# atx/padne

Hardware: AMD Instinct MI355X
Metric: CG solves/s (higher is better)
Workload: dtype f64; 1 GPU; C4 8-layer N=10M: 8-layer jittered triangular Laplacian, 9999392 nodes, via-ring stitched, 1 A source/sink, amg-PCG to rtol 1e-12; n_unknowns=9999391, nnz_per_rank=69955225, rows_per_rank=9999391, parallelism=layer-partitioned x1

## Files before the change

padne_amd/csrc/amg.hip:

```cpp
#include "common.hpp"

#include <functional>
#include <type_traits>
#include <memory>

#include <algorithm>
#include <chrono>
#include <math.h>
#include <stdlib.h>
#include <string.h>

namespace padne {

struct AmgLevel {
    const padne_csr *A = nullptr;
    padne_csr *A_owned = nullptr;
    padne_csr *P = nullptr;
    padne_csr *R = nullptr;
    padne_csr *W = nullptr;
    double lambda = 2.0;
    double jac = 0.0;
    long long n = 0;
    double *b = nullptr, *xa = nullptr, *xb = nullptr, *tmp = nullptr;
    float *b8 = nullptr, *xa8 = nullptr, *xb8 = nullptr, *tmp8 = nullptr;
// ... 183 lines not shown
            const double sgm = (off + fabs(dF)) / fabs(dF);
            my_max = sgm > my_max ? sgm : my_max;
            const double plain = abs_all * fabs(di);
            my_plain = plain > my_plain ? plain : my_plain;
        }
    }
    if (bound_partial != nullptr) {
        for (int o = 32; o > 0; o >>= 1) {
            my_max = fmax(my_max, __shfl_down(my_max, o, 64));
            my_plain = fmax(my_plain, __shfl_down(my_plain, o, 64));
        }
        if (lane == 0) {
            red[w] = my_max;
            red2[w] = my_plain;
        }
        __syncthreads();
        if (threadIdx.x == 0) {
            bound_partial[blockIdx.x] = fmax(fmax(red[0], red[1]), fmax(red[2], red[3]));
            bound_partial[kMaxPartials + blockIdx.x] = fmax(fmax(red2[0], red2[1]), fmax(red2[2], red2[3]));
        }
    }
}

template <typename T>
__global__ __launch_bounds__(256) void nbr_max(int n, int n_wtiles, const int *__restrict__ srow,
                                               const int *__restrict__ scol, const T *__restrict__ in,
                                               T *__restrict__ out) {
    constexpr int CH = 512;
    __shared__ T park_all[4 * CH];
    const int lane = threadIdx.x & 63, w = threadIdx.x >> 6;
    T *park = park_all + w * CH;
    const XcdSweep sw = xcd_sweep(n_wtiles, 4, w);
    for (long long wt = sw.t0; wt < sw.t1; wt += sw.stride) {
        const int row0 = (int)wt * 64;
        const int row1 = min(row0 + 64, n);
        const int r = row0 + lane;
        int rs = 0, re = 0;
        T m = 0;
        if (r < row1) {
            rs = srow[r];
            re = srow[r + 1];
            m = in[r];
        }
        const int k0 = __shfl(rs, 0, 64);
        const int k1 = __shfl(re, row1 - row0 - 1, 64);
        for (int base = k0; base < k1; base += CH) {
#pragma unroll
            for (int j = 0; j < CH / 64; ++j) {
                const int e = base + lane + 64 * j;
                park[lane + 64 * j] = (e < k1) ? in[scol[e]] : (T)0;
            }
            asm volatile("s_waitcnt lgkmcnt(0)" ::: "memory");
            __builtin_amdgcn_wave_barrier();
            const int lo = max(rs, base), hi = min(re, base + CH);
            for (int k = lo; k < hi; ++k) {
                const T v = park[k - base];
                m = v > m ? v : m;
            }
            asm volatile("" ::: "memory");
            __builtin_amdgcn_wave_barrier();
        }
        if (r < row1) out[r] = m;
    }
}

template <typename T>
__global__ __launch_bounds__(256) void nbr_max_wpr(int n, const int *__restrict__ srow, const int *__restrict__ scol,
                                                   const T *__restrict__ in, T *__restrict__ out) {
    const int lane = threadIdx.x & 63;
    const long long r = (long long)blockIdx.x * 4 + (threadIdx.x >> 6);
    if (r >= n) return;
    const int rs = srow[r], re = srow[r + 1];
    T m = in[r];
    for (int k = rs + lane; k < re; k += 64) {
        const T v = in[scol[k]];
        m = v > m ? v : m;
    }
#pragma unroll
    for (int off = 32; off > 0; off >>= 1) {
        const T o = __shfl_down(m, off, 64);
        m = o > m ? o : m;
    }
    if (lane == 0) out[r] = m;
}

__device__ __forceinline__ bool mis_decide_one(int i, unsigned int top, unsigned int *__restrict__ word,
                                               signed char *__restrict__ state) {
    const unsigned int mine = word[i];
    if (top == kMisRoot) {
        state[i] = 2;
        word[i] = 0u;
        return false;
    }
    if (top == mine) {
        state[i] = 1;
        word[i] = kMisRoot;
        return false;
    }
    return true;
}

template <typename T, bool DECIDE>
__global__ __launch_bounds__(256) void nbr_max_xw(int n, int n_wtiles, const int *__restrict__ srow,
                                                  const int *__restrict__ scol, const unsigned char *__restrict__ spos,
                                                  const int4 *__restrict__ xw_desc, const int run,
                                                  const T *__restrict__ in, T *__restrict__ out,
                                                  unsigned int *__restrict__ word, signed char *__restrict__ state,
                                                  int *__restrict__ undecided) {
    constexpr int CH = 512;
    __shared__ int open_red[4];
    int open = 0;
    __shared__ T park_all[4 * CH];
    __shared__ T xs_all[4 * 3 * 88];
    const int lane = threadIdx.x & 63, w = threadIdx.x >> 6;
    T *park = park_all + w * CH;
    T *xs = xs_all + w * 3 * 88;
    const XcdSweep sw = xcd_sweep(n_wtiles, 4, w);
    for (long long wt = sw.t0; wt < sw.t1; wt += sw.stride) {
        const int row0 = (int)wt * 64;
        const int row1 = min(row0 + 64, n);
        const int r = row0 + lane;
        int rs = 0, re = 0;
// ... 44 lines not shown
                for (int j = 0; j < CH / 64; ++j) {
                    const int e = base + lane + 64 * j;
                    park[lane + 64 * j] = (e < k1) ? in[scol[e]] : (T)0;
                }
                asm volatile("s_waitcnt lgkmcnt(0)" ::: "memory");
                __builtin_amdgcn_wave_barrier();
                const int lo = max(rs, base), hi = min(re, base + CH);
                for (int k = lo; k < hi; ++k) {
                    const T v = park[k - base];
                    m = v > m ? v : m;
                }
                asm volatile("" ::: "memory");
                __builtin_amdgcn_wave_barrier();
            }
        }
        if (r < row1) {
            if (DECIDE) {
                if (state[r] == 0 && mis_decide_one(r, (unsigned int)m, word, state)) ++open;
            } else {
                out[r] = m;
            }
        }
    }
    if (DECIDE) {
        for (int off = 32; off > 0; off >>= 1) open += __shfl_down(open, off, 64);
        if (lane == 0) open_red[w] = open;
        __syncthreads();
        if (threadIdx.x == 0) {
            const int t = open_red[0] + open_red[1] + open_red[2] + open_red[3];
            if (t) atomicAdd(undecided, t);
        }
    }
}

__global__ void mis_init_words(int n, unsigned int *__restrict__ word, signed char *__restrict__ state,
                               int *__restrict__ counters, int n_counters, unsigned char *__restrict__ pad, int n_pad) {
    const int i = blockIdx.x * blockDim.x + threadIdx.x;
    if (i < n) {
        word[i] = prio32_of(i);
        state[i] = 0;
    }
    if (i < n_counters) counters[i] = 0;
    if (pad != nullptr && i < n_pad) pad[i] = 0;
}

constexpr int kMisTailCap = 512;
__global__ __launch_bounds__(1024) void mis_tail_rounds(const int *__restrict__ cnt_ptr, int *list_a, int *list_b,
// ... 182 lines not shown
            for (int u = 0; u < 8; ++u) aj[u] = (k0 + u < k1 && j[u] != i) ? agg_in[j[u]] : -1;
#pragma unroll
            for (int u = 0; u < 8; ++u) {
                const double w = fabs(v[u]);
                if (aj[u] >= 0 && w > best) {
                    best = w;
                    a = aj[u];
                }
            }
        }
        for (int k = k0 + 8; k < k1; ++k) {
            const int j = scol[k];
            if (j == i) continue;
            const int aj = agg_in[j];
            if (aj < 0) continue;
            const double w = fabs(vals[k]);
            if (w > best) {
                best = w;
                a = aj;
            }
        }
    }
    agg_out[i] = a;
}

__global__ void flag_unaggregated(int n, const int *__restrict__ agg, int *__restrict__ flag) {
    const int i = blockIdx.x * blockDim.x + threadIdx.x;
    if (i < n) flag[i] = agg[i] < 0 ? 1 : 0;
}

__global__ void agg_singletons(int n, const int *__restrict__ scan, const long long *__restrict__ base_dev, int *__restrict__ agg) {
    const int i = blockIdx.x * blockDim.x + threadIdx.x;
    if (i < n && agg[i] < 0) agg[i] = (int)*base_dev + scan[i];
}

__global__ __launch_bounds__(256) void gershgorin_kernel(int n, const int *__restrict__ rowptr,
                                                         const double *__restrict__ vals,
                                                         const double *__restrict__ dinv,
                                                         double *__restrict__ partial_max) {
    __shared__ double red[256];
    double m = 0.0;
    for (int i = blockIdx.x * 256 + threadIdx.x; i < n; i += gridDim.x * 256) {
        double s = 0.0;
        for (int k = rowptr[i]; k < rowptr[i + 1]; ++k) s += fabs(vals[k]);
        s *= fabs(dinv[i]);
        m = s > m ? s : m;
// ... 1459 lines not shown
    PADNE_TRY(sc.alloc(&agg0, (size_t)n));
    PADNE_TRY(sc.alloc(&agg1, (size_t)n));
    constexpr int kMaxRounds = 256;
    PADNE_TRY(sc.alloc(&counter, (size_t)2 * kMaxRounds + 4));
    const dim3 g(nblk(n)), b(256);
    const int *srow = A->rowptr;
    int *scol = nullptr;
    PADNE_TRY(sc.alloc(&scol, (size_t)(A->nnz > 0 ? A->nnz : 1)));
    const int n_wt = (n + 63) / 64;
    int gm_x = std::min(2048, (n_wt + 3) / 4 > 0 ? (n_wt + 3) / 4 : 1);
    if (gm_x >= kNumXcd) gm_x -= gm_x % kNumXcd;
    const dim3 gm((unsigned)gm_x);
    double *bound_part = lambda_f != nullptr ? ctx->partials + 6 * kMaxPartials : nullptr;
    double *bound2 = nullptr;
    if (lambda_f != nullptr) PADNE_TRY(sc.alloc(&bound2, 2));
    const bool xw = A->xw_state == 1 && A->xw_run <= 85;
    unsigned char *spos = nullptr;
    if (xw) {
        PADNE_TRY(sc.alloc(&spos, (size_t)A->nnz + kPadNnz));
    }
    static_assert(kPadNnz >= 2 * kMaxRounds + 4, "one grid for everything the start clears");
    hipLaunchKernelGGL(mis_init_words, dim3(nblk(std::max(n, kPadNnz))), b, 0, s, n, w0, state, counter, 2 * kMaxRounds + 4,
                       spos != nullptr ? spos + A->nnz : (unsigned char *)nullptr, kPadNnz);
    hipLaunchKernelGGL(strength_mark, gm, b, 0, s, n, n_wt, A->rowptr, A->cols, A->vals, A->dinv, theta2, scol, bound_part,
                       xw ? A->xw_desc : (const int4 *)nullptr, xw ? (const unsigned char *)A->xw_lidx : (const unsigned char *)nullptr,
                       xw ? A->xw_run : 0, spos, vals32_out);
    PADNE_HIP_CHECK(hipGetLastError());
    const bool long_rows = !xw && n <= 65536 && A->nnz >= 24LL * n;
    auto launch_round = [&](int *open_counter) {
        if (xw) {
            hipLaunchKernelGGL((nbr_max_xw<unsigned int, false>), gm, b, 0, s, n, n_wt, srow, scol, spos, A->xw_desc, A->xw_run,
                               (const unsigned int *)w0, w1, (unsigned int *)nullptr, (signed char *)nullptr, (int *)nullptr);
            hipLaunchKernelGGL((nbr_max_xw<unsigned int, true>), gm, b, 0, s, n, n_wt, srow, scol, spos, A->xw_desc, A->xw_run,
                               (const unsigned int *)w1, (unsigned int *)nullptr, w0, state, open_counter);
        } else if (long_rows) {
            hipLaunchKernelGGL(nbr_max_wpr<unsigned int>, dim3((unsigned)((n + 3) / 4)), b, 0, s, n, srow, (const int *)scol,
                               (const unsigned int *)w0, w1);
            hipLaunchKernelGGL(nbr_max_wpr<unsigned int>, dim3((unsigned)((n + 3) / 4)), b, 0, s, n, srow, (const int *)scol,
                               (const unsigned int *)w1, w2);
            hipLaunchKernelGGL(mis_decide, dim3(std::min<unsigned>(g.x, 1024u)), b, 0, s, n, w0, w2, state, open_counter);
        } else {
            hipLaunchKernelGGL(nbr_max<unsigned int>, gm, b, 0, s, n, n_wt, srow, scol, w0, w1);
            hipLaunchKernelGGL(nbr_max<unsigned int>, gm, b, 0, s, n, n_wt, srow, scol, w1, w2);
            hipLaunchKernelGGL(mis_decide, dim3(std::min<unsigned>(g.x, 1024u)), b, 0, s, n, w0, w2, state, open_counter);
        }
    };
    if (lambda_f != nullptr)
        hipLaunchKernelGGL(fold_max2_kernel, dim3(1), dim3(256), 0, s, (const double *)bound_part,
                           (const double *)(bound_part + kMaxPartials), (int)gm.x, bound2);
    double h_bound2[2] = {0.0, 0.0};
    bool bound_pending = lambda_f != nullptr;
    auto count_back = [&](const int *dev_count, int *host_count) -> int {
        if (!bound_pending) return read_back(ctx, dev_count, sizeof(int), host_count);
        bound_pending = false;
        return read_back2(ctx, dev_count, sizeof(int), host_count, bound2, sizeof(h_bound2), h_bound2);
    };
    int open_count = n;
    int round = 0;
    const bool compact_ok = A->nnz <= 16LL * n;
    const int full_batch = n > 200000 ? 1 : 4;
    while (round < kMaxRounds && open_count > 0 && (!compact_ok || round < 2 || open_count > n / 8)) {
        const int reps = (round == 0 && compact_ok && full_batch < 2) ? 2 : full_batch;
        for (int rep = 0; rep < reps && round < kMaxRounds; ++rep, ++round) {
            launch_round(counter + round);
        }
        PADNE_HIP_CHECK(hipGetLastError());
        PADNE_TRY(count_back(counter + round - 1, &open_count));
    }
    if (open_count > 0) {
        int *list_a = (int *)w1, *list_b = (int *)w2;
        unsigned int *m2 = nullptr;
        PADNE_TRY(sc.alloc(&m2, (size_t)open_count));
        int *counters = counter + kMaxRounds;
        hipLaunchKernelGGL(mis_collect_open, dim3(std::min<unsigned>(g.x, 1024u)), b, 0, s, n, state, list_a, counters);
        PADNE_HIP_CHECK(hipGetLastError());
        int cnt = open_count, cur = 0;
        while (cur + 1 < kMaxRounds && cnt > 0) {
            if (cnt <= kMisTailCap) {
                hipLaunchKernelGGL(mis_tail_rounds, dim3(1), dim3(1024), 0, s, (const int *)(counters + cur), list_a, list_b, srow,
                                   (const int *)scol, w0, state, m2, counters + cur + 1, kMaxRounds - cur - 1);
                PADNE_HIP_CHECK(hipGetLastError());
                ++cur;
                round += kMaxRounds;
                PADNE_TRY(count_back(counters + cur, &cnt));
                break;
            }
            const dim3 gl(nblk(cnt));
// ... 3 lines not shown
                hipLaunchKernelGGL(mis_decide_list, gl, b, 0, s, counters + cur, list_a, m2, w0, state, list_b, counters + cur + 1);
                std::swap(list_a, list_b);
                ++cur;
            }
            PADNE_HIP_CHECK(hipGetLastError());
            PADNE_TRY(count_back(counters + cur, &cnt));
        }
        open_count = cnt;
    }
    PADNE_REQUIRE(open_count == 0, "independent-set rounds did not terminate");
    if (lambda_f != nullptr) {
        if (bound_pending) PADNE_TRY(read_back(ctx, bound2, sizeof(h_bound2), h_bound2));
        double m = h_bound2[0], mp = h_bound2[1];
        if (!(m > 0.0) || !(m < 1e6)) m = 2.0;
        if (!(mp > 0.0) || !(mp < 1e6)) mp = 2.0;
        *lambda_f = m;
        if (lambda_plain != nullptr) *lambda_plain = mp;
    }
    hipLaunchKernelGGL(flag_state, g, b, 0, s, n, state, flag, 1);
    ScanTicket t_roots, t_single;
    long long h_roots[2] = {0, 0}, h_single[2] = {0, 0};
    PADNE_TRY(scan_i32_begin(ctx, flag, scan, n, &t_roots, true));
    hipLaunchKernelGGL(agg_from_roots, g, b, 0, s, n, state, scan, agg0);
    hipLaunchKernelGGL(agg_join, g, b, 0, s, n, srow, scol, A->vals, agg0, agg1);
    hipLaunchKernelGGL(agg_join, g, b, 0, s, n, srow, scol, A->vals, agg1, agg0);
    hipLaunchKernelGGL(flag_unaggregated, g, b, 0, s, n, agg0, flag);
    int rc_scan = scan_i32_begin(ctx, flag, scan, n, &t_single, true);
    if (rc_scan == PADNE_OK && t_roots.bs != nullptr)
        hipLaunchKernelGGL(agg_singletons, g, b, 0, s, n, scan, (const long long *)(t_roots.bs + t_roots.nb), agg0);
    const int rc_roots = scan_i32_end(ctx, &t_roots, h_roots);
    if (rc_scan == PADNE_OK) rc_scan = scan_i32_end(ctx, &t_single, h_single);
    PADNE_TRY(rc_roots);
    PADNE_TRY(rc_scan);
    PADNE_HIP_CHECK(hipGetLastError());
    const long long n_roots = h_roots[0], n_single = h_single[0];
    PADNE_REQUIRE(n_roots >= 0 && n_single >= 0 && n_roots + n_single < 2147483647LL, "aggregate count out of range");
    *agg_out = agg0;
    *n_agg = (int)(n_roots + n_single);
    if (spos_out != nullptr) *spos_out = spos;
    if (scol_out != nullptr) *scol_out = scol;
    return PADNE_OK;
}

template <int CAP>
__global__ __launch_bounds__(128) void prolong_rows_lds(int n, const int *__restrict__ rowptr, const int *__restrict__ cols,
                                                        const double *__restrict__ vals, const double *__restrict__ dinv,
                                                        double theta2, double omega, const int *__restrict__ agg,
                                                        const int *__restrict__ slot_ptr, long long *__restrict__ key,
// ... 382 lines not shown
    bool valid = false;
    ~SlotRows() { release(); }
    void release() {
        if (ctx != nullptr) {
            pool_free(ctx, begin);
            pool_free(ctx, end);
            pool_free(ctx, key);
            pool_free(ctx, val);
        }
        begin = end = nullptr;
        key = nullptr;
        val = nullptr;
        valid = false;
    }
};

__global__ void slot_row_ends(int n, const int *__restrict__ slot_ptr, const int *__restrict__ row_len, int *__restrict__ end) {
    const int i = blockIdx.x * blockDim.x + threadIdx.x;
    if (i < n) end[i] = slot_ptr[i] + row_len[i];
}

static int spgemm(padne_ctx *ctx, const padne_csr *X, const padne_csr *Y, padne_csr **C, const SlotRows *y_slots = nullptr,
                  SlotRows *keep_slots = nullptr, const std::function<int()> *while_counting = nullptr,
                  const std::function<int()> *while_multiplying = nullptr) {
    const int *y_begin = y_slots != nullptr ? y_slots->begin : Y->rowptr;
    const int *y_end = y_slots != nullptr ? y_slots->end : Y->rowptr + 1;
    const int *y_cols = y_slots != nullptr ? (const int *)y_slots->key + 1 : Y->cols;
    const double *y_vals = y_slots != nullptr ? y_slots->val : Y->vals;
    const int y_cs = y_slots != nullptr ? 2 : 1;
    hipStream_t s = ctx->stream;
    Scratch sc(ctx);
    const int n = (int)X->n_rows;
    int *cnt = nullptr, *slot_ptr = nullptr, *row_len = nullptr;
    PADNE_TRY(sc.alloc(&cnt, (size_t)n + 1));
    PADNE_TRY(sc.alloc(&slot_ptr, (size_t)n + 1));
    PADNE_TRY(sc.alloc(&row_len, (size_t)n + 1));
    if (n > 0) {
        const double x_avg = (double)X->nnz / (double)n;
        if (x_avg > 48.0)
            hipLaunchKernelGGL((spgemm_count_lanes<32>), dim3(nblk((long long)n * 32)), dim3(256), 0, s, n, X->rowptr, X->cols, y_begin, y_end, cnt);
        else if (x_avg > 16.0)
            hipLaunchKernelGGL((spgemm_count_lanes<8>), dim3(nblk((long long)n * 8)), dim3(256), 0, s, n, X->rowptr, X->cols, y_begin, y_end, cnt);
        else
            hipLaunchKernelGGL(spgemm_count, dim3(nblk(n)), dim3(256), 0, s, n, X->rowptr, X->cols, y_begin, y_end, cnt);
    }
    PADNE_HIP_CHECK(hipGetLastError());
    int64_t n_slots = 0;
// ... 122 lines not shown
        keep_slots->release();
        int *end = (int *)pool_alloc(ctx, sizeof(int) * (size_t)(n > 0 ? n : 1));
        if (end == nullptr) return PADNE_E_NOMEM;
        int *first = row_begin != nullptr ? row_begin : slot_ptr;
        if (n > 0) hipLaunchKernelGGL(slot_row_ends, dim3(nblk(n)), dim3(256), 0, s, n, (const int *)first, row_len, end);
        PADNE_HIP_CHECK(hipGetLastError());
        keep_slots->ctx = ctx;
        keep_slots->n_rows = n;
        keep_slots->n_cols = Y->n_cols;
        keep_slots->n_slots = n_slots;
        keep_slots->begin = first;
        keep_slots->end = end;
        keep_slots->key = key;
        keep_slots->val = val;
        keep_slots->valid = true;
        sc.disown(first);
        sc.disown(key);
        sc.disown(val);
        if (C != nullptr) *C = nullptr;
        return PADNE_OK;
    }
    auto trampoline = [](void *f) -> int { return (*static_cast<const std::function<int()> *>(f))(); };
    return csr_from_slots(ctx, n, Y->n_cols, row_begin != nullptr ? row_begin : slot_ptr, key, val, row_len, C,
                          while_multiplying != nullptr ? +trampoline : nullptr, const_cast<std::function<int()> *>(while_multiplying));
}

__global__ void slot_row_lengths(int n, const int *__restrict__ begin, const int *__restrict__ end, int *__restrict__ len) {
    const int i = blockIdx.x * blockDim.x + threadIdx.x;
    if (i < n) len[i] = end[i] - begin[i];
}

__global__ __launch_bounds__(256) void w_from_slots_kernel(int n, const int *__restrict__ ap_begin,
                                                           const long long *__restrict__ ap_key,
                                                           const double *__restrict__ ap_val, const int *__restrict__ pr,
                                                           const int *__restrict__ pc, const double *__restrict__ pv,
                                                           const double *__restrict__ dinv, const double c,
                                                           const int *__restrict__ wr, int *__restrict__ wc,
                                                           float *__restrict__ wv) {
    __shared__ int rp_all[4][65];
    __shared__ int sp_all[4][65];
    const int lane = threadIdx.x & 63, w = threadIdx.x >> 6;
    int *rp = rp_all[w], *sp = sp_all[w];
    const long long n_wt = ((long long)n + 63) / 64;
    for (long long wt = (long long)blockIdx.x * 4 + w; wt < n_wt; wt += (long long)gridDim.x * 4) {
        const long long r0 = wt * 64;
        const int nr = (int)((n - r0) < 64 ? (n - r0) : 64);
        if (lane <= nr) rp[lane] = wr[r0 + lane];
// ... 337 lines not shown
        if ((rc = build_prolongator(ctx, A, agg, n_agg, omega, &L.P, spos, scol)) != PADNE_OK) { amg->levels.push_back(L); break; }
        pt.lap("prolongator");
        if (amg_verbose()) fprintf(stderr, "[amg]   P: %lld x %lld nnz=%lld\n", (long long)L.P->n_rows, (long long)L.P->n_cols, (long long)L.P->nnz);
        if (two && (rc = stream_order(ctx, aux)) != PADNE_OK) { amg->levels.push_back(L); break; }
        const std::function<int()> queue_transpose = [&]() -> int { return transpose(aux, L.P, &L.R); };
        SlotRows ap_rows;
        if ((rc = spgemm(ctx, A, L.P, &AP, nullptr, &ap_rows, &queue_transpose)) != PADNE_OK) { amg->levels.push_back(L); break; }
        if (L.R == nullptr && (rc = transpose(aux, L.P, &L.R)) != PADNE_OK) { amg->levels.push_back(L); break; }
        pt.lap("A*P (P^T queued beside it)");
        const bool with_w = lvl == 0 && want_f32 && ap_rows.valid && ctx->opt.amg_w >= 1;
        if (amg_verbose() && AP != nullptr) fprintf(stderr, "[amg]   AP nnz=%lld\n", (long long)AP->nnz);
        if (two && (rc = stream_order(aux, ctx)) != PADNE_OK) { if (AP) padne_csr_destroy(AP); amg->levels.push_back(L); break; }
        if (two && (rc = stream_order(ctx, aux)) != PADNE_OK) { if (AP) padne_csr_destroy(AP); amg->levels.push_back(L); break; }
        w_expected = with_w || (lvl > 0 && want_f32 && w_inner && ap_rows.valid);
        bool side_queued = false;
        const std::function<int()> queue_side = [&]() -> int {
            side_queued = true;
            if (with_w) {
                const double c0 = 1.0 / (0.5 * (L.lambda + L.lambda / kChebRatio));
                PADNE_TRY(build_w_operator(aux, A, L.P, ap_rows, ap_rows.n_slots, c0, &L.W));
            }
            return queue_level_extras(true);
        };
        if (ap_rows.valid) {
            padne_csr ap_shape;
            ap_shape.n_rows = ap_rows.n_rows;
            ap_shape.n_cols = ap_rows.n_cols;
            rc = spgemm(ctx, L.R, &ap_shape, &Ac, &ap_rows, nullptr, nullptr, &queue_side);
        } else {
            rc = spgemm(ctx, L.R, AP, &Ac, nullptr, nullptr, nullptr, &queue_side);
        }
        if (rc == PADNE_OK && !side_queued) rc = queue_side();
        if (rc != PADNE_OK && two) (void)hipStreamSynchronize(aux->stream);
        pt.lap("R*(AP)");
        if (amg_verbose() && rc == PADNE_OK) fprintf(stderr, "[amg]   Ac: n=%lld nnz=%lld\n", (long long)Ac->n_rows, (long long)Ac->nnz);
        if (AP) padne_csr_destroy(AP);
        auto take_slots = [](SlotRows &to, SlotRows &from) {
            std::swap(to.ctx, from.ctx);
            std::swap(to.begin, from.begin);
            std::swap(to.end, from.end);
            std::swap(to.key, from.key);
            std::swap(to.val, from.val);
            to.n_rows = from.n_rows;
            to.n_cols = from.n_cols;
            to.n_slots = from.n_slots;
            to.valid = from.valid;
        };
        if (with_w) {
            take_slots(ap_keep, ap_rows);
        } else if (lvl > 0 && rc == PADNE_OK && want_f32 && w_inner && ap_rows.valid) {
            ap_inner.emplace_back(new KeptSlots());
            ap_inner.back()->level = lvl;
            take_slots(ap_inner.back()->rows, ap_rows);
// ... 978 lines not shown
```

padne_amd/csrc/assemble.hip:

```cpp
#include "common.hpp"
#include "face.hpp"

#include <atomic>

#include <cmath>

#include <algorithm>

#include <string.h>

namespace padne {

constexpr int kScanItems = 16;
constexpr int kScanChunk = 256 * kScanItems;

__device__ __forceinline__ int block_exclusive_scan_256(int v, int *lds , int *total) {
    const int lane = threadIdx.x & 63, w = threadIdx.x >> 6;
    int inc = v;
#pragma unroll
    for (int off = 1; off < 64; off <<= 1) {
        const int t = __shfl_up(inc, off, 64);
        if (lane >= off) inc += t;
    }
    if (lane == 63) lds[w] = inc;
// ... 1442 lines not shown
        const int col = (int)(Kc[i][t] >> 32);
        double v = 0.0;
        while (i < n && (int)(Kc[i][t] >> 32) == col) {
            v = v + Vc[i][t];
            ++i;
        }
        if (v != 0.0) {
            key[s0 + o] = (long long)col << 32;
            val[s0 + o] = v;
            ++o;
        }
    }
    row_len[r] = o;
}

static int compact_rows_per_wave(long long n_rows, long long nnz) {
    if (n_rows <= 0 || n_rows > 100000 || nnz <= 16 * n_rows) return 64;
    return nnz <= 128 * n_rows ? 8 : 1;
}

__global__ __launch_bounds__(256) void compact_rows(long long n_rows, const int *__restrict__ slot_ptr,
                                                    const int *__restrict__ rowptr, const long long *__restrict__ key,
                                                    const double *__restrict__ val, int *__restrict__ cols,
                                                    double *__restrict__ vals, const int rpw) {
    __shared__ int rp_all[4][65];
    __shared__ int sp_all[4][65];
    const int lane = threadIdx.x & 63, w = threadIdx.x >> 6;
    int *rp = rp_all[w], *sp = sp_all[w];
    const long long n_wt = (n_rows + rpw - 1) / rpw;
    for (long long wt = (long long)blockIdx.x * 4 + w; wt < n_wt; wt += (long long)gridDim.x * 4) {
        const long long r0 = wt * rpw;
        const int nr = (int)((n_rows - r0) < rpw ? (n_rows - r0) : rpw);
        if (lane <= nr) rp[lane] = rowptr[r0 + lane];
        if (lane < nr) sp[lane] = slot_ptr[r0 + lane];
        if (lane == 0 && nr == 64) rp[64] = rowptr[r0 + 64];
        asm volatile("s_waitcnt lgkmcnt(0)" ::: "memory");
        __builtin_amdgcn_wave_barrier();
        const int d0 = rp[0], d1 = rp[nr];
        for (int k = d0 + lane; k < d1; k += 64) {
            int lo = 0, hi = nr;
            while (hi - lo > 1) {
                const int mid = (lo + hi) >> 1;
                if (rp[mid] <= k) lo = mid; else hi = mid;
            }
            const int src = sp[lo] + (k - rp[lo]);
            cols[k] = (int)(key[src] >> 32);
            vals[k] = val[src];
        }
        asm volatile("" ::: "memory");
        __builtin_amdgcn_wave_barrier();
    }
}

__global__ void fill_value_i32(int *p, long long n, int v) {
    const long long i = (long long)blockIdx.x * blockDim.x + threadIdx.x;
    if (i < n) p[i] = v;
}

__global__ void reduce_count(long long n_rows, const int *__restrict__ rowptr, const int *__restrict__ cols,
                             const int *__restrict__ map, const int *__restrict__ cmap, int *__restrict__ cnt) {
    const long long r = (long long)blockIdx.x * blockDim.x + threadIdx.x;
    if (r >= n_rows) return;
    const int t = map[r];
    if (t < 0) return;
    int c = 0;
    for (int k = rowptr[r]; k < rowptr[r + 1]; ++k) c += (cmap[cols[k]] >= 0) ? 1 : 0;
    if (c) atomicAdd(&cnt[t], c);
}

__global__ void reduce_fill(long long n_rows, const int *__restrict__ rowptr, const int *__restrict__ cols,
// ... 387 lines not shown
        padne_csr_destroy(m);
        return PADNE_E_HIP;
    }
    *out = m;
    return PADNE_OK;
}


int merge_slots_generic(padne_ctx *ctx, long long n_rows, const int *slot_ptr, long long *key, double *val,
                        int *row_len) {
    constexpr int kLdsCap = 32;
    hipLaunchKernelGGL(merge_rows_lds<kLdsCap>, dim3(nblk(n_rows, 128)), dim3(128), 0, ctx->stream, n_rows, slot_ptr, key,
                       val, row_len);
    hipLaunchKernelGGL(sort_long_rows_wave<kWaveSortCap>, dim3(std::min(nblk(n_rows, 256), 2048u)), dim3(256), 0, ctx->stream,
                       n_rows, (const int *)nullptr, slot_ptr, key, val, kLdsCap + 1, 0);
    hipLaunchKernelGGL(merge_rows<false>, dim3(nblk(n_rows, 128)), dim3(128), 0, ctx->stream, n_rows, 0LL, 0,
                       (const long long *)nullptr, (const double *)nullptr, slot_ptr, key, val, row_len,
                       (int *)nullptr, kLdsCap + 1, (const int *)nullptr, kWaveSortCap);
    PADNE_HIP_CHECK(hipGetLastError());
    return PADNE_OK;
}

int csr_from_slots(padne_ctx *ctx, long long n_rows, long long n_cols, const int *slot_ptr, const long long *key,
                   const double *val, const int *row_len, padne_csr **out, int (*while_scanning)(void *), void *while_scanning_arg) {
    hipStream_t s = ctx->stream;
    Scratch sc(ctx);
    int *rowptr_tmp = nullptr;
    PADNE_TRY(sc.alloc(&rowptr_tmp, (size_t)n_rows + 1));
    int64_t nnz = 0;
    {
        ScanTicket ticket;
        long long h[2] = {0, 0};
        PADNE_TRY(scan_i32_begin(ctx, row_len, rowptr_tmp, n_rows, &ticket, true));
        const int rc_cb = while_scanning != nullptr ? while_scanning(while_scanning_arg) : PADNE_OK;
        const int rc_scan = scan_i32_end(ctx, &ticket, h);
        PADNE_TRY(rc_cb);
        PADNE_TRY(rc_scan);
        if (h[0] < 0 || h[1] != 0) {
            set_error("scan of negative counts");
            return PADNE_E_INVALID;
        }
        if (h[0] >= 2147483647LL) {
            set_error("%lld entries exceed the 32-bit index space", h[0]);
            return PADNE_E_TOOLARGE;
        }
        nnz = h[0];
    }
    padne_csr *m = nullptr;
    PADNE_TRY(csr_alloc(ctx, n_rows, n_cols, nnz, &m));
    hipError_t e = hipMemcpyAsync(m->rowptr, rowptr_tmp, sizeof(int32_t) * (size_t)(n_rows + 1),
                                  hipMemcpyDeviceToDevice, s);
    if (e == hipSuccess && n_rows > 0) {
        const int rpw = compact_rows_per_wave(n_rows, nnz);
        hipLaunchKernelGGL(compact_rows, dim3(std::min(nblk((n_rows + rpw - 1) / rpw, 4), 65536u)), dim3(256), 0, s, n_rows, slot_ptr,
                           m->rowptr, key, val, m->cols, m->vals, rpw);
        e = hipGetLastError();
    }
    if (e != hipSuccess) {
        set_error("row compaction failed: %s", hipGetErrorString(e));
        padne_csr_destroy(m);
        return PADNE_E_HIP;
    }
    *out = m;
    return PADNE_OK;
}

__global__ void unpack_slots_kernel(long long nnz, const long long *__restrict__ key, const double *__restrict__ val,
                                    int *__restrict__ cols, double *__restrict__ vals) {
    for (long long k = (long long)blockIdx.x * blockDim.x + threadIdx.x; k < nnz; k += (long long)gridDim.x * blockDim.x) {
        cols[k] = (int)(key[k] >> 32);
        vals[k] = val[k];
    }
}

int sort_slots_exact(padne_ctx *ctx, long long n_rows, const int *slot_ptr, long long *key, double *val, int *row_len_scratch) {
    Scratch sc(ctx);
    int *long_list = nullptr;
    PADNE_TRY(sc.alloc(&long_list, (size_t)n_rows + 1));
// ... 711 lines not shown
```

padne_amd/csrc/capi.hip:

```cpp
#include "common.hpp"

#include <algorithm>

#include <math.h>
#include <stdarg.h>
#include <string.h>
#include <chrono>

namespace padne {

std::atomic<long long> g_launch_count{0};

void options_from_env(padne_options *o) {
    *o = padne_options();
    auto on = [](const char *name) { const char *e = getenv(name); return e != nullptr && e[0] != '\0' && !(e[0] == '0' && e[1] == '\0'); };
    auto has = [](const char *list, const char *word) {
        const size_t n = strlen(word);
        for (const char *p = list; p != nullptr && *p != '\0';) {
            const char *q = strchr(p, ',');
            const size_t len = q != nullptr ? (size_t)(q - p) : strlen(p);
            if (len >= n && strncmp(p, word, n) == 0 && (len == n || p[n] == ':')) return p;
            p = q != nullptr ? q + 1 : nullptr;
        }
        return (const char *)nullptr;
// ... 5 lines not shown
    o->pcg_no_xhist = on("PADNE_PCG_NO_XHIST");
    o->gj_vector = on("PADNE_GJ_VECTOR");
    o->no_batch = on("PADNE_NO_BATCH");
    o->no_mailbox = on("PADNE_NO_MAILBOX");
    o->no_p2p = on("PADNE_NO_P2P");
    o->no_split = on("PADNE_NO_SPLIT");
    o->no_xwindow = on("PADNE_NO_XWINDOW");
    o->setup_one_stream = on("PADNE_SETUP_ONE_STREAM");
    if (const char *e = getenv("PADNE_CG_SINGLE_REDUCTION")) o->cg_single_reduction = atoi(e) != 0 ? 1 : 0;
    if (const char *e = getenv("PADNE_LOCKSTEP_NARROW")) o->lockstep_narrow = atoi(e);
    if (const char *e = getenv("PADNE_AMG_COARSE_N")) o->amg_coarse_n = std::min(4096, std::max(16, atoi(e)));
    if (const char *e = getenv("PADNE_AMG_GATHER_N")) o->amg_gather_n = atoll(e);
    if (const char *e = getenv("PADNE_P2P_TIMEOUT_MS")) {
        const long v = atol(e);
        if (v > 0 && v <= 600000) o->p2p_timeout_ms = (unsigned)v;
    }
    if (const char *f = getenv("PADNE_FORCE")) {
        o->force_asm_hash = has(f, "asm_hash") != nullptr;
        o->force_asm_two_pass = has(f, "asm_two_pass") != nullptr;
        o->force_relabel_slots = has(f, "relabel_slots") != nullptr;
        o->force_transpose_cursors = has(f, "transpose_cursors") != nullptr;
        o->force_xhist_small = has(f, "xhist_small") != nullptr;
        o->force_relabel_lanes = has(f, "relabel_lanes") != nullptr;
        if (const char *w = has(f, "spgemm_split")) o->force_spgemm_split = w[12] == ':' ? atoll(w + 13) : 30000;
    }
    if (const char *v = getenv("PADNE_VERBOSE")) {
        o->verbose_amg = has(v, "amg") != nullptr;
        o->verbose_xw = has(v, "xw") != nullptr;
        o->verbose_pool = has(v, "pool") != nullptr;
    }
}

static thread_local char g_err[1024] = "";

void set_error(const char *fmt, ...) {
    va_list ap;
    va_start(ap, fmt);
    vsnprintf(g_err, sizeof(g_err), fmt, ap);
    va_end(ap);
}

int ensure_workspace(padne_ctx *ctx, size_t bytes) {
    if (ctx->ws_bytes >= bytes) return PADNE_OK;
    if (ctx->ws) {
        PADNE_HIP_CHECK(hipStreamSynchronize(ctx->stream));
        PADNE_HIP_CHECK(hipFree(ctx->ws));
// ... 557 lines not shown
```

padne_amd/csrc/common.hpp:

```cpp
#pragma once

#include <hip/hip_runtime.h>
#include <stdint.h>
#include <stdio.h>
#include <map>
#include <string>
#include <unordered_map>
#include <vector>

#include "../../include/padne_hip.h"
#include "../../include/padne_hip_test.h"
#include "../../include/padne_hip_probe.h"

#include <atomic>

namespace padne {

extern std::atomic<long long> g_launch_count;

void set_error(const char *fmt, ...);

#define PADNE_HIP_CHECK(expr)                                                              \
    do {                                                                                   \
        hipError_t _e = (expr);                                                            \
// ... 72 lines not shown
};

struct padne_options {
    bool amg_f64 = false;
    int amg_w = 2;
    bool amg_exchange_all = false;
    bool pcg_p64 = false;
    bool pcg_no_xhist = false;
    bool gj_vector = false;
    bool no_batch = false;
    bool no_mailbox = false;
    bool no_p2p = false;
    bool no_split = false;
    bool no_xwindow = false;
    bool setup_one_stream = false;
    int cg_single_reduction = -1;
    int lockstep_narrow = -1;
    int amg_coarse_n = 2048;
    long long amg_gather_n = 0;
    unsigned p2p_timeout_ms = 20000;
    bool force_asm_hash = false, force_asm_two_pass = false, force_relabel_slots = false, force_transpose_cursors = false;
    bool force_relabel_lanes = false;
    bool force_xhist_small = false;
    long long force_spgemm_split = 0;
    bool verbose_amg = false, verbose_xw = false, verbose_pool = false;
};
namespace padne { void options_from_env(padne_options *o); }

struct padne_ctx {
    int device = 0;
    padne_options opt;
    hipStream_t stream = nullptr;
    double *partials = nullptr;
    double *scalars = nullptr;
    int32_t *status = nullptr;
    void *pinned = nullptr;
    void *ws = nullptr;
    size_t ws_bytes = 0;
    void *comm = nullptr;
    void *team = nullptr;
    int rank = 0, world = 1;
    bool halo_on = false;
    long long halo_n_owned = 0;
    int halo_m = 0, halo_n_export = 0;
    int32_t *halo_export = nullptr;
    void *p2p_mbox = nullptr;
// ... 170 lines not shown
        for (void *p : ptrs) if (p) pool_free(ctx, p);
        ptrs.clear();
    }
    void disown(void *p) {
        for (void *&q : ptrs) if (q == p) q = nullptr;
    }
    template <typename T> int alloc(T **out, size_t count) {
        void *p = pool_alloc(ctx, sizeof(T) * (count ? count : 1));
        if (p == nullptr) return PADNE_E_NOMEM;
        ptrs.push_back(p);
        *out = (T *)p;
        return PADNE_OK;
    }
};
static inline unsigned nblk(long long n, int bs = 256) {
    const long long b = (n + bs - 1) / bs;
    return (unsigned)(b > 0 ? b : 1);
}
int merge_slots_generic(padne_ctx *ctx, long long n_rows, const int *slot_ptr, long long *key, double *val,
                        int *row_len);
int sort_slots_exact(padne_ctx *ctx, long long n_rows, const int *slot_ptr, long long *key, double *val, int *row_len_scratch);
int csr_from_slots(padne_ctx *ctx, long long n_rows, long long n_cols, const int *slot_ptr, const long long *key,
                   const double *val, const int *row_len, padne_csr **out,
                   int (*while_scanning)(void *) = nullptr, void *while_scanning_arg = nullptr);
int csr_from_exact_slots(padne_ctx *ctx, long long n_rows, long long n_cols, long long nnz, const int *slot_ptr,
                         const long long *key, const double *val, padne_csr **out);

}
```

Before: 32.00 solves/s.

## Fuse MIS decide into neighbour-max, add wave-per-row kernels for small coarse levels

Fuses the second neighbour-max pass with the MIS decide step, which removes one kernel launch and one buffer round-trip per round. It skips the undecided-count atomic on rounds that are not read back. For small, dense coarse levels it adds grid-stride wave-per-row kernels for strength marking and aggregate joining, and it computes the coarse-matrix inverse diagonal during CSR compaction. All of this targets AMG setup cost on the coarse levels, which is likely a small share of the time per solve if setup is not timed per solve.

```diff
diff --git a/padne_amd/csrc/amg.hip b/padne_amd/csrc/amg.hip
--- a/padne_amd/csrc/amg.hip
+++ b/padne_amd/csrc/amg.hip
@@ -229,12 +229,104 @@
     }
 }
 
-template <typename T>
+__global__ __launch_bounds__(256) void strength_mark_wpr(int n, const int *__restrict__ rowptr, const int *__restrict__ cols,
+                                                         const double *__restrict__ vals, const double *__restrict__ dinv,
+                                                         double theta2, int *__restrict__ scol, double *__restrict__ bound_partial,
+                                                         float *__restrict__ vals32) {
+    constexpr int CH = 512;
+    __shared__ unsigned char fl_all[4 * CH];
+    __shared__ double pv_all[4 * CH];
+    __shared__ double red[4], red2[4];
+    const int lane = threadIdx.x & 63, w = threadIdx.x >> 6;
+    unsigned char *fl = fl_all + w * CH;
+    double *pv = pv_all + w * CH;
+    double my_max = 0.0, my_plain = 0.0;
+    for (long long rr = (long long)blockIdx.x * 4 + w; rr < n; rr += (long long)gridDim.x * 4) {
+        const int r = (int)rr;
+        const int rs = rowptr[r], re = rowptr[r + 1];
+        const double di = dinv[r];
+        double dF = 1.0 / di, off_strong = 0.0, off_all = 0.0, abs_all = 0.0;
+        for (int base = rs; base < re; base += CH) {
+            const int hi = min(re, base + CH);
+            for (int e = base + lane; e < hi; e += 64) {
+                const int c = cols[e];
+                const double v = vals[e];
+                if (vals32 != nullptr) vals32[e] = (float)v;
+                const bool st = c != r && strong(v, di, dinv[c], theta2);
+                scol[e] = st ? c : r;
+                if (bound_partial != nullptr) {
+                    fl[e - base] = (unsigned char)((c == r ? 0x40 : 0) | (st ? 0x80 : 0));
+                    pv[e - base] = v;
+                }
+            }
+            if (bound_partial != nullptr) {
+                asm volatile("s_waitcnt lgkmcnt(0)" ::: "memory");
+                __builtin_amdgcn_wave_barrier();
+                if (lane == 0) {
+                    for (int k = base; k < hi; ++k) {
+                        const unsigned char f = fl[k - base];
+                        const double v = pv[k - base];
+                        abs_all += fabs(v);
+                        if (f & 0x40) continue;
+                        off_all += fabs(v);
+                        if (f & 0x80) off_strong += fabs(v);
+                        else dF += v;
+                    }
+                }
+            }
+            asm volatile("" ::: "memory");
+            __builtin_amdgcn_wave_barrier();
+        }
+        if (bound_partial != nullptr && lane == 0) {
+            double off = off_strong;
+            if (!(dF * di > 0.05)) {
+                dF = 1.0 / di;
+                off = off_all;
+            }
+            const double sgm = (off + fabs(dF)) / fabs(dF);
+            my_max = sgm > my_max ? sgm : my_max;
+            const double plain = abs_all * fabs(di);
+            my_plain = plain > my_plain ? plain : my_plain;
+        }
+    }
+    if (bound_partial != nullptr) {
+        if (lane == 0) {
+            red[w] = my_max;
+            red2[w] = my_plain;
+        }
+        __syncthreads();
+        if (threadIdx.x == 0) {
+            bound_partial[blockIdx.x] = fmax(fmax(red[0], red[1]), fmax(red[2], red[3]));
+            bound_partial[kMaxPartials + blockIdx.x] = fmax(fmax(red2[0], red2[1]), fmax(red2[2], red2[3]));
+        }
+    }
+}
+
+__device__ __forceinline__ bool mis_decide_one(int i, unsigned int top, unsigned int *__restrict__ word,
+                                               signed char *__restrict__ state) {
+    const unsigned int mine = word[i];
+    if (top == kMisRoot) {
+        state[i] = 2;
+        word[i] = 0u;
+        return false;
+    }
+    if (top == mine) {
+        state[i] = 1;
+        word[i] = kMisRoot;
+        return false;
+    }
+    return true;
+}
+
+template <typename T, bool DECIDE = false>
 __global__ __launch_bounds__(256) void nbr_max(int n, int n_wtiles, const int *__restrict__ srow,
                                                const int *__restrict__ scol, const T *__restrict__ in,
-                                               T *__restrict__ out) {
+                                               T *__restrict__ out, unsigned int *__restrict__ word = nullptr,
+                                               signed char *__restrict__ state = nullptr, int *__restrict__ undecided = nullptr) {
     constexpr int CH = 512;
     __shared__ T park_all[4 * CH];
+    __shared__ int open_red[4];
+    int open = 0;
     const int lane = threadIdx.x & 63, w = threadIdx.x >> 6;
     T *park = park_all + w * CH;
     const XcdSweep sw = xcd_sweep(n_wtiles, 4, w);
@@ -267,44 +359,61 @@
             asm volatile("" ::: "memory");
             __builtin_amdgcn_wave_barrier();
         }
-        if (r < row1) out[r] = m;
-    }
-}
-
-template <typename T>
+        if (r < row1) {
+            if (DECIDE) {
+                if (state[r] == 0 && mis_decide_one(r, (unsigned int)m, word, state)) ++open;
+            } else {
+                out[r] = m;
+            }
+        }
+    }
+    if (DECIDE && undecided != nullptr) {
+        for (int off = 32; off > 0; off >>= 1) open += __shfl_down(open, off, 64);
+        if (lane == 0) open_red[w] = open;
+        __syncthreads();
+        if (threadIdx.x == 0) {
+            const int t = open_red[0] + open_red[1] + open_red[2] + open_red[3];
+            if (t) atomicAdd(undecided, t);
+        }
+    }
+}
+
+template <typename T, bool DECIDE = false>
 __global__ __launch_bounds__(256) void nbr_max_wpr(int n, const int *__restrict__ srow, const int *__restrict__ scol,
-                                                   const T *__restrict__ in, T *__restrict__ out) {
-    const int lane = threadIdx.x & 63;
-    const long long r = (long long)blockIdx.x * 4 + (threadIdx.x >> 6);
-    if (r >= n) return;
-    const int rs = srow[r], re = srow[r + 1];
-    T m = in[r];
-    for (int k = rs + lane; k < re; k += 64) {
-        const T v = in[scol[k]];
-        m = v > m ? v : m;
-    }
-#pragma unroll
-    for (int off = 32; off > 0; off >>= 1) {
-        const T o = __shfl_down(m, off, 64);
-        m = o > m ? o : m;
-    }
-    if (lane == 0) out[r] = m;
-}
-
-__device__ __forceinline__ bool mis_decide_one(int i, unsigned int top, unsigned int *__restrict__ word,
-                                               signed char *__restrict__ state) {
-    const unsigned int mine = word[i];
-    if (top == kMisRoot) {
-        state[i] = 2;
-        word[i] = 0u;
-        return false;
-    }
-    if (top == mine) {
-        state[i] = 1;
-        word[i] = kMisRoot;
-        return false;
-    }
-    return true;
+                                                   const T *__restrict__ in, T *__restrict__ out,
+                                                   unsigned int *__restrict__ word = nullptr, signed char *__restrict__ state = nullptr,
+                                                   int *__restrict__ undecided = nullptr) {
+    __shared__ int open_red[4];
+    const int lane = threadIdx.x & 63, w = threadIdx.x >> 6;
+    int open = 0;
+    for (long long r = (long long)blockIdx.x * 4 + w; r < n; r += (long long)gridDim.x * 4) {
+        const int rs = srow[r], re = srow[r + 1];
+        T m = in[r];
+        for (int k = rs + lane; k < re; k += 64) {
+            const T v = in[scol[k]];
+            m = v > m ? v : m;
+        }
+#pragma unroll
+        for (int off = 32; off > 0; off >>= 1) {
+            const T o = __shfl_down(m, off, 64);
+            m = o > m ? o : m;
+        }
+        if (lane == 0) {
+            if (DECIDE) {
+                if (state[r] == 0 && mis_decide_one((int)r, (unsigned int)m, word, state)) ++open;
+            } else {
+                out[r] = m;
+            }
+        }
+    }
+    if (DECIDE && undecided != nullptr) {
+        if (lane == 0) open_red[w] = open;
+        __syncthreads();
+        if (threadIdx.x == 0) {
+            const int t = open_red[0] + open_red[1] + open_red[2] + open_red[3];
+            if (t) atomicAdd(undecided, t);
+        }
+    }
 }
 
 template <typename T, bool DECIDE>
@@ -395,7 +504,7 @@
             }
         }
     }
-    if (DECIDE) {
+    if (DECIDE && undecided != nullptr) {
         for (int off = 32; off > 0; off >>= 1) open += __shfl_down(open, off, 64);
         if (lane == 0) open_red[w] = open;
         __syncthreads();
@@ -624,6 +733,44 @@
         }
     }
     agg_out[i] = a;
+}
+
+__global__ __launch_bounds__(256) void agg_join_wpr(int n, const int *__restrict__ srow, const int *__restrict__ scol,
+                                                    const double *__restrict__ vals, const int *__restrict__ agg_in,
+                                                    int *__restrict__ agg_out) {
+    const int lane = threadIdx.x & 63, w = threadIdx.x >> 6;
+    for (long long rr = (long long)blockIdx.x * 4 + w; rr < n; rr += (long long)gridDim.x * 4) {
+        const int i = (int)rr;
+        int a = agg_in[i];
+        if (a < 0) {
+            double best = -1.0;
+            int bk = 0x7fffffff;
+            const int k1 = srow[i + 1];
+            for (int k = srow[i] + lane; k < k1; k += 64) {
+                const int j = scol[k];
+                if (j == i) continue;
+                const int aj = agg_in[j];
+                if (aj < 0) continue;
+                const double wt = fabs(vals[k]);
+                if (wt > best) {
+                    best = wt;
+                    bk = k;
+                    a = aj;
+                }
+            }
+#pragma unroll
+            for (int off = 32; off > 0; off >>= 1) {
+                const double ob = __shfl_down(best, off, 64);
+                const int ok = __shfl_down(bk, off, 64), oa = __shfl_down(a, off, 64);
+                if (ob > best || (ob == best && ok < bk)) {
+                    best = ob;
+                    bk = ok;
+                    a = oa;
+                }
+            }
+        }
+        if (lane == 0) agg_out[i] = a;
+    }
 }
 
 __global__ void flag_unaggregated(int n, const int *__restrict__ agg, int *__restrict__ flag) {
@@ -2129,11 +2276,19 @@
     static_assert(kPadNnz >= 2 * kMaxRounds + 4, "one grid for everything the start clears");
     hipLaunchKernelGGL(mis_init_words, dim3(nblk(std::max(n, kPadNnz))), b, 0, s, n, w0, state, counter, 2 * kMaxRounds + 4,
                        spos != nullptr ? spos + A->nnz : (unsigned char *)nullptr, kPadNnz);
-    hipLaunchKernelGGL(strength_mark, gm, b, 0, s, n, n_wt, A->rowptr, A->cols, A->vals, A->dinv, theta2, scol, bound_part,
-                       xw ? A->xw_desc : (const int4 *)nullptr, xw ? (const unsigned char *)A->xw_lidx : (const unsigned char *)nullptr,
-                       xw ? A->xw_run : 0, spos, vals32_out);
+    const bool long_rows = !xw && n <= 65536 && A->nnz >= 24LL * n;
+    const bool small_old = ctx->opt.force_small_level_rows;
+    const bool fused_decide = !small_old;
+    const bool rows_wpr = long_rows && !small_old;
+    const dim3 gw(std::min<unsigned>((unsigned)((n + 3) / 4), 1024u));
+    static_assert(kMaxPartials >= 1024, "a bound per workgroup of strength_mark_wpr");
+    if (rows_wpr)
+        hipLaunchKernelGGL(strength_mark_wpr, gw, b, 0, s, n, A->rowptr, A->cols, A->vals, A->dinv, theta2, scol, bound_part, vals32_out);
+    else
+        hipLaunchKernelGGL(strength_mark, gm, b, 0, s, n, n_wt, A->rowptr, A->cols, A->vals, A->dinv, theta2, scol, bound_part,
+                           xw ? A->xw_desc : (const int4 *)nullptr, xw ? (const unsigned char *)A->xw_lidx : (const unsigned char *)nullptr,
+                           xw ? A->xw_run : 0, spos, vals32_out);
     PADNE_HIP_CHECK(hipGetLastError());
-    const bool long_rows = !xw && n <= 65536 && A->nnz >= 24LL * n;
     auto launch_round = [&](int *open_counter) {
         if (xw) {
             hipLaunchKernelGGL((nbr_max_xw<unsigned int, false>), gm, b, 0, s, n, n_wt, srow, scol, spos, A->xw_desc, A->xw_run,
@@ -2143,9 +2298,18 @@
         } else if (long_rows) {
             hipLaunchKernelGGL(nbr_max_wpr<unsigned int>, dim3((unsigned)((n + 3) / 4)), b, 0, s, n, srow, (const int *)scol,
                                (const unsigned int *)w0, w1);
+            if (fused_decide) {
+                hipLaunchKernelGGL((nbr_max_wpr<unsigned int, true>), gw, b, 0, s, n,
+                                   srow, (const int *)scol, (const unsigned int *)w1, (unsigned int *)nullptr, w0, state, open_counter);
+                return;
+            }
             hipLaunchKernelGGL(nbr_max_wpr<unsigned int>, dim3((unsigned)((n + 3) / 4)), b, 0, s, n, srow, (const int *)scol,
                                (const unsigned int *)w1, w2);
             hipLaunchKernelGGL(mis_decide, dim3(std::min<unsigned>(g.x, 1024u)), b, 0, s, n, w0, w2, state, open_counter);
+        } else if (fused_decide) {
+            hipLaunchKernelGGL(nbr_max<unsigned int>, gm, b, 0, s, n, n_wt, srow, scol, w0, w1);
+            hipLaunchKernelGGL((nbr_max<unsigned int, true>), gm, b, 0, s, n, n_wt, srow, (const int *)scol, (const unsigned int *)w1,
+                               (unsigned int *)nullptr, w0, state, open_counter);
         } else {
             hipLaunchKernelGGL(nbr_max<unsigned int>, gm, b, 0, s, n, n_wt, srow, scol, w0, w1);
             hipLaunchKernelGGL(nbr_max<unsigned int>, gm, b, 0, s, n, n_wt, srow, scol, w1, w2);
@@ -2154,7 +2318,7 @@
     };
     if (lambda_f != nullptr)
         hipLaunchKernelGGL(fold_max2_kernel, dim3(1), dim3(256), 0, s, (const double *)bound_part,
-                           (const double *)(bound_part + kMaxPartials), (int)gm.x, bound2);
+                           (const double *)(bound_part + kMaxPartials), (int)(rows_wpr ? gw.x : gm.x), bound2);
     double h_bound2[2] = {0.0, 0.0};
     bool bound_pending = lambda_f != nullptr;
     auto count_back = [&](const int *dev_count, int *host_count) -> int {
@@ -2169,7 +2333,8 @@
     while (round < kMaxRounds && open_count > 0 && (!compact_ok || round < 2 || open_count > n / 8)) {
         const int reps = (round == 0 && compact_ok && full_batch < 2) ? 2 : full_batch;
         for (int rep = 0; rep < reps && round < kMaxRounds; ++rep, ++round) {
-            launch_round(counter + round);
+            const bool counted = small_old || rep + 1 == reps || round + 1 == kMaxRounds;
+            launch_round(counted ? counter + round : (int *)nullptr);
         }
         PADNE_HIP_CHECK(hipGetLastError());
         PADNE_TRY(count_back(counter + round - 1, &open_count));
@@ -2219,8 +2384,13 @@
     long long h_roots[2] = {0, 0}, h_single[2] = {0, 0};
     PADNE_TRY(scan_i32_begin(ctx, flag, scan, n, &t_roots, true));
     hipLaunchKernelGGL(agg_from_roots, g, b, 0, s, n, state, scan, agg0);
-    hipLaunchKernelGGL(agg_join, g, b, 0, s, n, srow, scol, A->vals, agg0, agg1);
-    hipLaunchKernelGGL(agg_join, g, b, 0, s, n, srow, scol, A->vals, agg1, agg0);
+    if (rows_wpr) {
+        hipLaunchKernelGGL(agg_join_wpr, gw, b, 0, s, n, srow, (const int *)scol, (const double *)A->vals, (const int *)agg0, agg1);
+        hipLaunchKernelGGL(agg_join_wpr, gw, b, 0, s, n, srow, (const int *)scol, (const double *)A->vals, (const int *)agg1, agg0);
+    } else {
+        hipLaunchKernelGGL(agg_join, g, b, 0, s, n, srow, scol, A->vals, agg0, agg1);
+        hipLaunchKernelGGL(agg_join, g, b, 0, s, n, srow, scol, A->vals, agg1, agg0);
+    }
     hipLaunchKernelGGL(flag_unaggregated, g, b, 0, s, n, agg0, flag);
     int rc_scan = scan_i32_begin(ctx, flag, scan, n, &t_single, true);
     if (rc_scan == PADNE_OK && t_roots.bs != nullptr)
@@ -2649,7 +2819,7 @@
 
 static int spgemm(padne_ctx *ctx, const padne_csr *X, const padne_csr *Y, padne_csr **C, const SlotRows *y_slots = nullptr,
                   SlotRows *keep_slots = nullptr, const std::function<int()> *while_counting = nullptr,
-                  const std::function<int()> *while_multiplying = nullptr) {
+                  const std::function<int()> *while_multiplying = nullptr, const bool with_dinv = false) {
     const int *y_begin = y_slots != nullptr ? y_slots->begin : Y->rowptr;
     const int *y_end = y_slots != nullptr ? y_slots->end : Y->rowptr + 1;
     const int *y_cols = y_slots != nullptr ? (const int *)y_slots->key + 1 : Y->cols;
@@ -2818,7 +2988,8 @@
     }
     auto trampoline = [](void *f) -> int { return (*static_cast<const std::function<int()> *>(f))(); };
     return csr_from_slots(ctx, n, Y->n_cols, row_begin != nullptr ? row_begin : slot_ptr, key, val, row_len, C,
-                          while_multiplying != nullptr ? +trampoline : nullptr, const_cast<std::function<int()> *>(while_multiplying));
+                          while_multiplying != nullptr ? +trampoline : nullptr, const_cast<std::function<int()> *>(while_multiplying),
+                          with_dinv);
 }
 
 __global__ void slot_row_lengths(int n, const int *__restrict__ begin, const int *__restrict__ end, int *__restrict__ len) {
@@ -3202,13 +3373,14 @@
             }
             return queue_level_extras(true);
         };
+        const bool dinv_from_compaction = !ctx->opt.force_small_level_rows;
         if (ap_rows.valid) {
             padne_csr ap_shape;
             ap_shape.n_rows = ap_rows.n_rows;
             ap_shape.n_cols = ap_rows.n_cols;
-            rc = spgemm(ctx, L.R, &ap_shape, &Ac, &ap_rows, nullptr, nullptr, &queue_side);
+            rc = spgemm(ctx, L.R, &ap_shape, &Ac, &ap_rows, nullptr, nullptr, &queue_side, dinv_from_compaction);
         } else {
-            rc = spgemm(ctx, L.R, AP, &Ac, nullptr, nullptr, nullptr, &queue_side);
+            rc = spgemm(ctx, L.R, AP, &Ac, nullptr, nullptr, nullptr, &queue_side, dinv_from_compaction);
         }
         if (rc == PADNE_OK && !side_queued) rc = queue_side();
         if (rc != PADNE_OK && two) (void)hipStreamSynchronize(aux->stream);
diff --git a/padne_amd/csrc/assemble.hip b/padne_amd/csrc/assemble.hip
--- a/padne_amd/csrc/assemble.hip
+++ b/padne_amd/csrc/assemble.hip
@@ -1488,11 +1488,12 @@
 __global__ __launch_bounds__(256) void compact_rows(long long n_rows, const int *__restrict__ slot_ptr,
                                                     const int *__restrict__ rowptr, const long long *__restrict__ key,
                                                     const double *__restrict__ val, int *__restrict__ cols,
-                                                    double *__restrict__ vals, const int rpw) {
+                                                    double *__restrict__ vals, const int rpw, double *__restrict__ dinv = nullptr) {
     __shared__ int rp_all[4][65];
     __shared__ int sp_all[4][65];
+    __shared__ int hd_all[4][64];
     const int lane = threadIdx.x & 63, w = threadIdx.x >> 6;
-    int *rp = rp_all[w], *sp = sp_all[w];
+    int *rp = rp_all[w], *sp = sp_all[w], *hd = hd_all[w];
     const long long n_wt = (n_rows + rpw - 1) / rpw;
     for (long long wt = (long long)blockIdx.x * 4 + w; wt < n_wt; wt += (long long)gridDim.x * 4) {
         const long long r0 = wt * rpw;
@@ -1500,6 +1501,7 @@
         if (lane <= nr) rp[lane] = rowptr[r0 + lane];
         if (lane < nr) sp[lane] = slot_ptr[r0 + lane];
         if (lane == 0 && nr == 64) rp[64] = rowptr[r0 + 64];
+        if (dinv != nullptr) hd[lane] = 0;
         asm volatile("s_waitcnt lgkmcnt(0)" ::: "memory");
         __builtin_amdgcn_wave_barrier();
         const int d0 = rp[0], d1 = rp[nr];
@@ -1510,8 +1512,20 @@
                 if (rp[mid] <= k) lo = mid; else hi = mid;
             }
             const int src = sp[lo] + (k - rp[lo]);
-            cols[k] = (int)(key[src] >> 32);
-            vals[k] = val[src];
+            const int c = (int)(key[src] >> 32);
+            const double v = val[src];
+            cols[k] = c;
+            vals[k] = v;
+            if (dinv != nullptr && (long long)c == r0 + lo) {
+                dinv[r0 + lo] = 1.0 / (0.0 + v);
+                hd[lo] = 1;
+            }
+        }
+        if (dinv != nullptr) {
+            asm volatile("s_waitcnt lgkmcnt(0)" ::: "memory");
+            __builtin_amdgcn_wave_barrier();
+            const double zero = 0.0;
+            if (lane < nr && hd[lane] == 0) dinv[r0 + lane] = 1.0 / zero;
         }
         asm volatile("" ::: "memory");
         __builtin_amdgcn_wave_barrier();
@@ -1945,7 +1959,8 @@
 }
 
 int csr_from_slots(padne_ctx *ctx, long long n_rows, long long n_cols, const int *slot_ptr, const long long *key,
-                   const double *val, const int *row_len, padne_csr **out, int (*while_scanning)(void *), void *while_scanning_arg) {
+                   const double *val, const int *row_len, padne_csr **out, int (*while_scanning)(void *), void *while_scanning_arg,
+                   bool with_dinv) {
     hipStream_t s = ctx->stream;
     Scratch sc(ctx);
     int *rowptr_tmp = nullptr;
@@ -1973,10 +1988,17 @@
     PADNE_TRY(csr_alloc(ctx, n_rows, n_cols, nnz, &m));
     hipError_t e = hipMemcpyAsync(m->rowptr, rowptr_tmp, sizeof(int32_t) * (size_t)(n_rows + 1),
                                   hipMemcpyDeviceToDevice, s);
+    if (e == hipSuccess && with_dinv && n_rows > 0 && n_rows <= n_cols && m->dinv == nullptr) {
+        m->dinv = (double *)pool_alloc(m->owner ? m->owner : ctx, sizeof(double) * (size_t)n_rows);
+        if (m->dinv == nullptr) {
+            padne_csr_destroy(m);
+            return PADNE_E_NOMEM;
+        }
+    }
     if (e == hipSuccess && n_rows > 0) {
         const int rpw = compact_rows_per_wave(n_rows, nnz);
         hipLaunchKernelGGL(compact_rows, dim3(std::min(nblk((n_rows + rpw - 1) / rpw, 4), 65536u)), dim3(256), 0, s, n_rows, slot_ptr,
-                           m->rowptr, key, val, m->cols, m->vals, rpw);
+                           m->rowptr, key, val, m->cols, m->vals, rpw, with_dinv ? m->dinv : (double *)nullptr);
         e = hipGetLastError();
     }
     if (e != hipSuccess) {
diff --git a/padne_amd/csrc/capi.hip b/padne_amd/csrc/capi.hip
--- a/padne_amd/csrc/capi.hip
+++ b/padne_amd/csrc/capi.hip
@@ -51,6 +51,7 @@
         o->force_transpose_cursors = has(f, "transpose_cursors") != nullptr;
         o->force_xhist_small = has(f, "xhist_small") != nullptr;
         o->force_relabel_lanes = has(f, "relabel_lanes") != nullptr;
+        o->force_small_level_rows = has(f, "small_level_rows") != nullptr;
         if (const char *w = has(f, "spgemm_split")) o->force_spgemm_split = w[12] == ':' ? atoll(w + 13) : 30000;
     }
     if (const char *v = getenv("PADNE_VERBOSE")) {
diff --git a/padne_amd/csrc/common.hpp b/padne_amd/csrc/common.hpp
--- a/padne_amd/csrc/common.hpp
+++ b/padne_amd/csrc/common.hpp
@@ -118,6 +118,7 @@
     bool force_asm_hash = false, force_asm_two_pass = false, force_relabel_slots = false, force_transpose_cursors = false;
     bool force_relabel_lanes = false;
     bool force_xhist_small = false;
+    bool force_small_level_rows = false;
     long long force_spgemm_split = 0;
     bool verbose_amg = false, verbose_xw = false, verbose_pool = false;
 };
@@ -334,7 +335,7 @@
 int sort_slots_exact(padne_ctx *ctx, long long n_rows, const int *slot_ptr, long long *key, double *val, int *row_len_scratch);
 int csr_from_slots(padne_ctx *ctx, long long n_rows, long long n_cols, const int *slot_ptr, const long long *key,
                    const double *val, const int *row_len, padne_csr **out,
-                   int (*while_scanning)(void *) = nullptr, void *while_scanning_arg = nullptr);
+                   int (*while_scanning)(void *) = nullptr, void *while_scanning_arg = nullptr, bool with_dinv = false);
 int csr_from_exact_slots(padne_ctx *ctx, long long n_rows, long long n_cols, long long nnz, const int *slot_ptr,
                          const long long *key, const double *val, padne_csr **out);
 
```

Result: slower. 31.46 solves/s (-1.7%).
